# TencentYoutuResearch/ImageMatching-OETR

Hardware: AMD Instinct MI355X
Metric: image-pairs/sec @640x640 (OETR hot path: feature correlation + overlap regression, features resident in HBM) (higher is better)
Workload: dtype f32 (3xf16-split operands, fp32 accumulate); 1 GPU; BASELINE configs[1]: batch=8 pairs/GPU, 640x640 -> 20x20 tokens/image, C=256, 8 enc + 2 dec layers, f32_split_f16; pairs_per_gpu=8, global_pairs=8, streams=3, world_size=1, gpu_max_hw_queues=4, encoder_tile_rows=64, tail_mode=direct form (throughput setting for overlapped streams), parallelism=pairs sharded over 1 rank(s); all-gather of boxes only

## Files before the change

imagematching_oetr_amd/csrc/api.hip:

```cpp
#include <math.h>
#include <stdlib.h>
#include <string.h>

#include <string>
#include <vector>

#include "../../include/oetr_hip.h"
#include "common.h"

using namespace oetr;

constexpr int OETR_PREREDUCE_MIN_TOKENS = 768;
constexpr int OETR_DIRECT_TAIL_MIN_ROWS = 16000;

namespace {

thread_local std::string g_err;

oetr_status fail(oetr_status st, const std::string& msg) {
  g_err = msg;
  return st;
}
oetr_status hip_fail(hipError_t e, const char* what) {
  return fail(OETR_ERR_HIP, std::string(what) + ": " + hipGetErrorString(e));
// ... 91 lines not shown
    "k_decoder", "k_heat_conv", "k_heat_final", "k_size_reg", "k_boxes", "k_decoder_convp",
    "k_heat_combine", "k_neck_proj", "k_neck_conv", "k_neck_out", "k_kv_reduce"};

struct oetr_trace {
  std::vector<hipEvent_t> ev;
  std::vector<int> kid;
  int used = 0;
  int dropped = 0;
};

struct oetr_ctx {
  oetr_trace* trace = nullptr;
  int device = 0;
  int mode = GM_SPLIT;
  int kv_prereduce = -1;
  mutable int dec_fault = 0;
  int dec_split = 0;
  int tail_mode = 0;
  int policy = 0;
  int enc_tile = 0;
  int attn_full = 0;
  int num_cus = 256;
  float* dev = nullptr;
  size_t dev_floats = 0;
  EncLayerDev enc[OETR_N_ENC];
  DecKVDev dkv;
  DecLayerDev dec[OETR_N_DEC];
  const float* qe[2];
  const float *dec_tgt1, *dec_q0, *dec_qkv1;
  HeadsDev heads;
// ... 30 lines not shown

bool make_geom(int n, int hf1, int wf1, int hf2, int wf2, Geom* g) {
  if (n <= 0 || hf1 <= 0 || wf1 <= 0 || hf2 <= 0 || wf2 <= 0) return false;
  const long L1 = (long)hf1 * wf1, L2 = (long)hf2 * wf2;
  if (L1 > OETR_MAX_TOKENS || L2 > OETR_MAX_TOKENS) return false;
  if ((long)n * (L1 + L2) > (1L << 30) / C) return false;
  g->N = n;
  g->L[0] = (int)L1; g->L[1] = (int)L2;
  g->hf[0] = hf1; g->wf[0] = wf1; g->hf[1] = hf2; g->wf[1] = wf2;
  g->nt[0] = (g->L[0] + TM - 1) / TM; g->nt[1] = (g->L[1] + TM - 1) / TM;
  g->row0[0] = 0; g->row0[1] = n * g->L[0];
  g->prow0[0] = 0; g->prow0[1] = g->L[0];
  g->tile0[0] = 0; g->tile0[1] = n * g->nt[0];
  g->ntiles = n * (g->nt[0] + g->nt[1]);
  g->rows = n * (g->L[0] + g->L[1]);
  return true;
}

int encoder_tile_rows(const oetr_ctx* h, const Geom& g) {
  if (!gm_half(h->mode) || h->attn_full) return TM;
  const int want = h->enc_tile;
  if (want == TM || want == 64) return want;
  return g.ntiles > h->num_cus ? 64 : TM;
}
Geom encoder_geom(const Geom& g, int rows) {
  Geom e = g;
  for (int i = 0; i < 2; ++i) e.nt[i] = (g.L[i] + rows - 1) / rows;
  e.tile0[0] = 0; e.tile0[1] = g.N * e.nt[0];
  e.ntiles = g.N * (e.nt[0] + e.nt[1]);
  return e;
}

Workspace carve(const Geom& g, void* base, bool attn_full = false) {
  Workspace w;
  size_t off = 0;
  auto take = [&](size_t floats) {
    float* p = base ? reinterpret_cast<float*>(static_cast<char*>(base) + off) : nullptr;
    off += (floats * sizeof(float) + 255) & ~size_t(255);
    return p;
  };
  const size_t rows = g.rows, nt = g.ntiles;
  w.flags = reinterpret_cast<uint32_t*>(take(OETR_WORKSPACE_STATUS_BYTES / sizeof(float)));
  w.x = take(rows * C);
  w.qp = take((rows + (size_t)2 * g.N * 64) * C);
  w.pos = take((size_t)(g.L[0] + g.L[1]) * C);
// ... 119 lines not shown

oetr_status run_correlation(oetr_ctx* h, const Geom& g, const Workspace& w, const float* feat1,
                            const float* feat2, const float* pos1, const float* pos2,
                            int enc_layers, hipStream_t s, bool with_decoder = true,
                            bool resident = false, const float* mask1 = nullptr,
                            const float* mask2 = nullptr) {
  EncLaunch p;
  memset(&p, 0, sizeof(p));
  if (!resident) {
    p.feat_nchw[0] = feat1; p.feat_nchw[1] = feat2;
    p.pos_nchw[0] = pos1; p.pos_nchw[1] = pos2;
    p.pos_out = w.pos;
  }
  p.tile_rows = encoder_tile_rows(h, g);
  p.g = encoder_geom(g, p.tile_rows);
#ifdef OETR_ABLATE
  { const char* e = getenv("OETR_ABLATE"); p.dbg = e ? atoi(e) : 0; }
#endif
#ifdef OETR_PHASE_TIMING
  {
    static long long* tb = nullptr;
    if (!tb) (void)hipMalloc(&tb, sizeof(long long) * 16 * 65536);
    p.tbuf = tb;
    g_tbuf = tb;
  }
#endif
  p.x = w.x; p.qp = w.qp; p.pos = w.pos;
  p.mask[0] = mask1; p.mask[1] = mask2;
  p.flags = w.flags;
  p.attn_full = h->attn_full;
// ... 1000 lines not shown
    return fail(OETR_ERR_BAD_ARG, "oetr_debug_mfma_rate: NULL output or seconds outside (0, 30]");
  int ndev = 0;
  if (hipGetDeviceCount(&ndev) != hipSuccess || ndev <= 0 || device < 0 || device >= ndev)
    return fail(OETR_ERR_NO_DEVICE, "no HIP device " + std::to_string(device));
  hipDeviceProp_t prop;
  HIP_TRY(hipGetDeviceProperties(&prop, device));
  int prev = 0;
  (void)hipGetDevice(&prev);
  hipError_t e = hipSetDevice(device);
  if (e == hipSuccess) e = measure_mfma_rate(prop.multiProcessorCount, seconds, tflops, static_cast<hipStream_t>(stream));
  (void)hipSetDevice(prev);
  if (e != hipSuccess) return hip_fail(e, "oetr_debug_mfma_rate");
  return OETR_OK;
}

oetr_status oetr_set_state_prereduce(oetr_handle h, int on) {
  if (!h) return fail(OETR_ERR_BAD_ARG, "oetr_set_state_prereduce: NULL handle");
  if (on < -1 || on > 1) return fail(OETR_ERR_BAD_ARG, "oetr_set_state_prereduce: -1 (auto), 0 (off) or 1 (a reduction launch between the encoder launches)");
  h->kv_prereduce = on;
  return OETR_OK;
}

oetr_status oetr_set_attention(oetr_handle h, oetr_attention mode) {
  if (!h) return fail(OETR_ERR_BAD_ARG, "oetr_set_attention: NULL handle");
  if (mode != OETR_ATTENTION_LINEAR && mode != OETR_ATTENTION_FULL)
    return fail(OETR_ERR_BAD_ARG, "oetr_set_attention: unknown mode");
  if (mode == OETR_ATTENTION_FULL && h->policy != 0)
    return fail(OETR_ERR_UNSUPPORTED, "attention 'full' is not built for OETR_DTYPE_F32_SPLIT_QK16");
  if (mode == OETR_ATTENTION_FULL && !gm_f16_range(h->mode) && h->mode != GM_F32)
    return fail(OETR_ERR_UNSUPPORTED, "attention 'full' is built for OETR_DTYPE_F32_SPLIT_F16, OETR_DTYPE_F16 and OETR_DTYPE_F32");
// ... 46 lines not shown
```

imagematching_oetr_amd/csrc/common.h:

```cpp
#pragma once
#include <hip/hip_runtime.h>
#include <stdint.h>

#include <type_traits>

namespace oetr {

constexpr int C = 256;
constexpr int NH = 8;
constexpr int HD = 32;
constexpr int FF = 512;
constexpr int TM = 32;
constexpr int LDA = C + 4;
constexpr int LDH = FF + 4;
constexpr int NTHREADS = 256;
constexpr int KV_FLOATS = NH * HD * HD;
constexpr float LN_EPS = 1e-5f;
constexpr float ATTN_EPS = 1e-6f;
constexpr int MAX_TOKENS = 10000;


#ifdef OETR_ABLATE
#define ABL(flags, bit) (((flags) & (bit)) != 0)
#else
// ... 46 lines not shown
template <> struct SitePolicy<0> {
  static constexpr int Q = SITE_FULL, K = SITE_FULL, V = SITE_FULL, MERGE = SITE_FULL, MLP1 = SITE_FULL,
                       MLP2 = SITE_FULL, DEC_K = SITE_FULL, DEC_V = SITE_FULL;
};
template <> struct SitePolicy<1> {
  static constexpr int Q = SITE_HI, K = SITE_HI, V = SITE_FULL, MERGE = SITE_FULL, MLP1 = SITE_FULL,
                       MLP2 = SITE_FULL, DEC_K = SITE_HI, DEC_V = SITE_FULL;
};
constexpr int N_POLICIES = 2;

constexpr float SPLIT_SCALE = 2048.0f;
constexpr float SPLIT_INV = 1.0f / 2048.0f;
constexpr int LDAH = C + 8;
constexpr int LDHH = FF + 8;

struct Geom {
  int N;
  int L[2];
  int hf[2], wf[2];
  int nt[2];
  int row0[2];
  int prow0[2];
  int tile0[2];
  int ntiles;
  int rows;
};

#if defined(__HIPCC__)

__device__ __forceinline__ float wave_max(float v) {
#pragma unroll
  for (int off = 32; off > 0; off >>= 1) v = fmaxf(v, __shfl_xor(v, off, 64));
  return v;
}

__device__ __forceinline__ int crow(int r, int half) {
  return (r & 3) + 8 * (r >> 2) + 4 * half;
}

__device__ __forceinline__ float exp_neg(float x) {
  const float L2E_HI = 1.4426950216293335f, L2E_LO = 1.9259629911266175e-08f;
// ... 61 lines not shown
  const f32x2 w1 = f32x2{fminf(a1[0], GELU_T), fminf(a1[1], GELU_T)};
  f32x2 q0 = splat2(GELU_Q[GELU_DEG]), q1 = splat2(GELU_Q[GELU_DEG]);
#pragma unroll
  for (int i = GELU_DEG - 1; i >= 0; --i) {
    q0 = __builtin_elementwise_fma(q0, w0, splat2(GELU_Q[i]));
    q1 = __builtin_elementwise_fma(q1, w1, splat2(GELU_Q[i]));
  }
  const f32x2 u0 = __builtin_elementwise_fma(w0, q0, splat2(-1.0f));
  const f32x2 u1 = __builtin_elementwise_fma(w1, q1, splat2(-1.0f));
  f32x4 g;
  g[0] = fmaf(-fabsf(v[0]), __builtin_amdgcn_exp2f(u0[0]), fmaxf(v[0], 0.f));
  g[2] = fmaf(-fabsf(v[2]), __builtin_amdgcn_exp2f(u1[0]), fmaxf(v[2], 0.f));
  g[1] = fmaf(-fabsf(v[1]), __builtin_amdgcn_exp2f(u0[1]), fmaxf(v[1], 0.f));
  g[3] = fmaf(-fabsf(v[3]), __builtin_amdgcn_exp2f(u1[1]), fmaxf(v[3], 0.f));
  return g;
}

__device__ __forceinline__ int xcd_remap(int bid, int nwg) {
  const int q = nwg >> 3, r = nwg & 7, xcd = bid & 7, idx = bid >> 3;
  return (xcd < r ? xcd * (q + 1) : r * (q + 1) + (xcd - r) * q) + idx;
}

template <int NT, int U>
struct GemmRegs {
  f32x4 b[U][NT];
  f32x4 a[U];
};

template <int NT, int U>
__device__ __forceinline__ void gemm_fetch(GemmRegs<NT, U>& r, const float* a_ptr,
                                           const f32x4* const (&w_ptr)[NT], int chunk, unsigned ln) {
#pragma unroll
  for (int u = 0; u < U; ++u)
#pragma unroll
    for (int t = 0; t < NT; ++t) r.b[u][t] = w_ptr[t][(chunk * U + u) * 64 + ln];
// ... 796 lines not shown
```

imagematching_oetr_amd/csrc/encoder.hip:

```cpp
#include <type_traits>

#include "common.h"


#ifndef OETR_SOAK_AMP
#define OETR_SOAK_AMP 0
#endif
#ifndef OETR_SPLIT_STATE
#define OETR_SPLIT_STATE 1
#endif

namespace oetr {

constexpr int S0_OFF = 0;
constexpr int S1_OFF = S0_OFF + TM * LDA;
constexpr int H_OFF = S1_OFF + TILE_FLOATS;
constexpr int KSUM_OFF = H_OFF + HID_FLOATS;
constexpr int Z_OFF = KSUM_OFF + C;
constexpr int LNP_OFF = Z_OFF + TM * NH;
constexpr int SMEM_FLOATS = LNP_OFF + 6 * C;

template <int NW>
struct EncCfg {
  static constexpr int NT = 8 / NW;
// ... 687 lines not shown
          if (lane == 0) p.z0_out[(size_t)slot * NH + h] = z;
        }
      }
    };
    dec_layer(std::integral_constant<int, 0>{});
    dec_layer(std::integral_constant<int, 1>{});
  }
  range_report<MODE>(rg, p.flags);
}

constexpr int LNX_LD = 36;
template <int RTW>
struct E2 {
  static constexpr int RFL = (2 * RTW * LDAH * 2 + 3) / 4;
  static_assert(RFL >= RTW * LDA, "region holds the f32 tile too");
  static constexpr int R1 = 0, R2 = RFL, KSUM = 2 * RFL, LNP = KSUM + C;
  static constexpr int LNX = LNP + 6 * C;
  static constexpr int SMEM = LNX + RTW * LNX_LD;
};

template <int MODE, int NMT = 2, bool MASKED = false>
__device__ __forceinline__ void kv_state_64(const f32x16 (&accK)[NMT], const f32x16 (&accV)[NMT],
                                            int S_len, int nvalid, int half, bool two, f32x16& kv,
                                            float& ksum, Range& rg, const float* msk_s = nullptr) {
  const float inv_len = 1.0f / (float)S_len;
  kv = f32x16{0};
  ksum = 0.f;
  int nv2 = nvalid - 4 * half;
  asm volatile("" : "+v"(nv2));
  if constexpr (MODE == GM_SPLIT && OETR_SPLIT_STATE) {
    f32x16 c1 = {0};
#if OETR_SOAK_AMP & 2
    __builtin_amdgcn_s_setprio(3);
#endif
    auto row_tile = [&](auto MT_) {
      constexpr int mt = decltype(MT_)::value;
#pragma unroll
      for (int st = 0; st < 2; ++st) {
        f32x4 k0, k1, v0, v1;
#pragma unroll
        for (int i = 0; i < 8; ++i) {
          const int r = 8 * st + i;
          float m;
          if constexpr (MASKED) m = msk_s[32 * mt + crow(r, half)];
          else m = 32 * mt + crow(r, 0) < nv2 ? 1.0f : 0.0f;
          const float kk = elu1(accK[mt][r]) * m;
          const float vv = accV[mt][r] * (inv_len * m);
          ksum += kk;
          if (i < 4) { k0[i] = kk; v0[i] = vv; } else { k1[i - 4] = kk; v1[i - 4] = vv; }
        }
        f32x4 ah, al, bh, bl;
        split8(k0, k1, ah, al, rg);
        split8(v0, v1, bh, bl, rg);
        mma16_split3(ah, al, bh, bl, kv, c1);
        __builtin_amdgcn_sched_barrier(0);
      }
    };
    row_tile(std::integral_constant<int, 0>{});
    if constexpr (NMT == 2) {
      if (two) row_tile(std::integral_constant<int, 1>{});
    }
#if OETR_SOAK_AMP & 2
    __builtin_amdgcn_s_setprio(0);
#endif
#pragma unroll
    for (int r = 0; r < 16; ++r) kv[r] = fmaf(c1[r], SPLIT_INV, kv[r]);
  } else {
    auto row_tile = [&](auto MT_) {
      constexpr int mt = decltype(MT_)::value;
      auto operands = [&](int r, float& k, float& v) {
        float m;
        if constexpr (MASKED) m = msk_s[32 * mt + crow(r, half)];
        else m = 32 * mt + crow(r, 0) < nv2 ? 1.0f : 0.0f;
        const float x = accK[mt][r];
        k = (elu1(x)) * m;
        ksum += k;
        v = accV[mt][r] * (inv_len * m);
      };
      float kc, vc;
      operands(0, kc, vc);
#pragma unroll
      for (int r = 0; r < 16; ++r) {
        float kn = 0.f, vn = 0.f;
        if (r + 1 < 16) operands(r + 1, kn, vn);
        kv = __builtin_amdgcn_mfma_f32_32x32x2f32(kc, vc, kv, 0, 0, 0);
        __builtin_amdgcn_sched_barrier(0);
        kc = kn; vc = vn;
// ... 32 lines not shown
  float* lnp_s = smem + L2::LNP;
  float* lnx_s = smem + L2::LNX;
  using WS = WStream2T<MODE, ROWS, NMT>;
  WS ws;
  constexpr int P_MERGE = 0;
  constexpr int P_1A = WS::adv(P_MERGE), P_1B = WS::adv(P_1A), P_2A = WS::adv(P_1B), P_2B = WS::adv(P_2A);
  constexpr int P_T0 = HAS_B ? WS::adv(P_2B) : 0;
  constexpr int P_T1 = WS::adv(P_T0), P_T2 = WS::adv(P_T1), P_T3 = WS::adv(P_T2);

  const Geom& g = p.g;
  const int tid = threadIdx.x, lane = tid & 63, wave = __builtin_amdgcn_readfirstlane(tid >> 6);
  const int half = lane >> 5, col = lane & 31;
  const int wcol = 32 * wave;
  const int lrow = tid / TPR, lpart = tid % TPR;

  const int logical = xcd_remap(blockIdx.x, g.ntiles);
  const int per = g.nt[0] + g.nt[1];
  const int n = logical / per;
  const int rem = logical - n * per;
  const int side = rem >= g.nt[0];
  const int t_idx = side ? rem - g.nt[0] : rem;
  const int L = g.L[side];
  const int l0 = t_idx * RTW;
  const int nvalid = min(RTW, L - l0);
  const size_t row_base = (size_t)g.row0[side] + (size_t)n * L + l0;
  const int slot = g.tile0[side] + n * g.nt[side] + t_idx;
  const size_t qrow_base = (size_t)slot * RTW;
  const bool nchw = !HAS_B && p.feat_nchw[0] != nullptr;
  ws.set_rows(nvalid);
  ws.set_lane(lane);

  stage_ln_params<THREADS, HAS_B, TAIL>(lnp_s, p, tid);
  const f32x4* pos = reinterpret_cast<const f32x4*>(
                         p.pos + (size_t)(g.prow0[side] + l0 + min(lrow, nvalid - 1)) * C) + lpart;

  f32x16 xacc[NMT];
  PHASE_STAMP(p, 0);
  if (!HAS_B) PHASE_STAMP(p, 13);

  if (HAS_B) {
    const int ss = p.b_cross ? 1 - side : side;
    const int S_len = g.L[ss];
    const int nts = p.kv_reduced ? 1 : g.nt[ss];
    const int src_slot0 = p.kv_reduced ? ss * g.N + n : g.tile0[ss] + n * g.nt[ss];

    f32x4 kvB[4];
#pragma unroll
    for (int q = 0; q < 4; ++q) kvB[q] = f32x4{0.f, 0.f, 0.f, 0.f};
    {
      constexpr int KVR = 7;
      const unsigned ln = lane, kl = tid & (C - 1);
      const f32x4* kvp = reinterpret_cast<const f32x4*>(p.kv_in) + ((size_t)src_slot0 * NH + wave) * 256;
      const float* ksp = p.ks_in + (size_t)src_slot0 * C;
      float ks = 0.f;
      if (nts == 1) {
#pragma unroll
        for (int e = 0; e < 4; ++e) kvB[e] = kvp[e * 64 + ln];
        ks = ksp[kl];
      } else
      for (int ti0 = 0; ti0 < nts; ti0 += KVR) {
        f32x4 tmp[KVR][4];
        float kt[KVR];
#pragma unroll
        for (int u = 0; u < KVR; ++u) {
          const int ti = min(ti0 + u, nts - 1);
#pragma unroll
          for (int e = 0; e < 4; ++e) tmp[u][e] = kvp[(size_t)ti * (NH * 256) + e * 64 + ln];
          kt[u] = ksp[(size_t)ti * C + kl];
        }
#pragma unroll
        for (int u = 0; u < KVR; ++u)
          if (ti0 + u < nts) {
#pragma unroll
            for (int e = 0; e < 4; ++e) kvB[e] += tmp[u][e];
            ks += kt[u];
          }
      }
      if (tid < C) ksum_s[tid] = ks;
    }
    ws.template prime<C, P_MERGE, SP::MERGE>(p.b.wmerge, p.b.wmerge_l, wave, 0, lane);
    f32x4 qfrag[NMT][4];
    {
      const f32x4* qf = reinterpret_cast<const f32x4*>(p.qp + qrow_base * C) + (size_t)wave * NMT * 4 * 64;
#pragma unroll
      for (int mt = 0; mt < NMT; ++mt)
#pragma unroll
        for (int u = 0; u < 4; ++u) qfrag[mt][u] = qf[(mt * 4 + u) * 64 + (unsigned)lane];
    }
#pragma unroll
    for (int mt = 0; mt < NMT; ++mt) {
      const float* xr = p.x + (row_base + min(32 * mt + col, nvalid - 1)) * C + wcol + 4 * half;
#pragma unroll
      for (int g4 = 0; g4 < 4; ++g4) {
        const f32x4 v = *reinterpret_cast<const f32x4*>(xr + 8 * g4);
#pragma unroll
        for (int i = 0; i < 4; ++i) xacc[mt][4 * g4 + i] = v[i];
      }
    }
    __syncthreads();
    PHASE_STAMP(p, 1);

    {
      f32x4 kvh[2], kvl[2], ksh[2], ksl[2];
      const float inv_S = 1.0f / (float)S_len;
      (void)inv_S;
      if constexpr (gm_f16_range(MODE)) {
#pragma unroll
        for (int s2 = 0; s2 < 2; ++s2) {
          split8(kvB[2 * s2], kvB[2 * s2 + 1], kvh[s2], kvl[s2], rg);
          const float* kr = ksum_s + wave * HD + 4 * half + 16 * s2;
          split8(*reinterpret_cast<const f32x4*>(kr) * inv_S, *reinterpret_cast<const f32x4*>(kr + 8) * inv_S,
                 ksh[s2], ksl[s2], rg);
        }
      }
#pragma unroll
      for (int mt = 0; mt < NMT; ++mt) {
        if (mt == 1 && !ws.two()) break;
// ... 113 lines not shown
      PHASE_STAMP(p, 7);
      ws.template gemm<FF, P_2B, (TAIL != 2), C, SP::MLP2, SNEXT, XTR>(P1, p.b.w2, p.b.w2_l, wave, 16, lane, xacc,
                                                                       TAIL == 0 ? p.a.wq : p.d.wk[0],
                                                                       TAIL == 0 ? p.a.wq_l : p.d.wk_l[0], wave, 0);
    }
#pragma unroll
    for (int mt = 0; mt < NMT; ++mt)
#pragma unroll
      for (int g4 = 0; g4 < 4; ++g4)
        *reinterpret_cast<f32x4*>(Xf + (32 * mt + col) * LDA + wcol + 8 * g4 + 4 * half) =
            f32x4{xacc[mt][4 * g4], xacc[mt][4 * g4 + 1], xacc[mt][4 * g4 + 2], xacc[mt][4 * g4 + 3]};
    __syncthreads();
#pragma unroll
    for (int i = 0; i < RTW / 8; ++i) {
      const int r = wave + 8 * i;
      if (r < nvalid)
        store16(p.x + (row_base + r) * C, 16u * (unsigned)lane,
                                    *reinterpret_cast<const f32x4*>(Xf + r * LDA + 4 * lane));
    }
    PHASE_STAMP(p, 8);
    if (TAIL == 2) { range_report<MODE>(rg, p.flags); return; }
  } else {
    if (nchw) {
      load_tile_nchw<THREADS, RTW>(R1f, p.feat_nchw[side] + (size_t)n * C * L + l0, L, nvalid, tid);
      load_tile_nchw<THREADS, RTW>(R2f, p.pos_nchw[side] + l0, L, nvalid, tid);
    } else {
#pragma unroll
      for (int i = 0; i < (RTW * C / 4) / THREADS; ++i) {
        const int idx = tid + THREADS * i;
        const int r = idx >> 6, c4 = idx & 63;
        *reinterpret_cast<f32x4*>(R1f + r * LDA + 4 * c4) =
            reinterpret_cast<const f32x4*>(p.x + (row_base + min(r, nvalid - 1)) * C)[c4];
      }
    }
    if (TAIL == 0) ws.template prime<C, P_T0, SP::Q>(p.a.wq, p.a.wq_l, wave, 0, lane);
    if (TAIL == 1) ws.template prime<C, P_T0, SP::DEC_K>(p.d.wk[0], p.d.wk_l[0], wave, 0, lane);
    __syncthreads();
    if (nchw) {
      store_tile_tokens<THREADS, RTW>(p.x + row_base * C, R1f, nvalid, tid);
      if (n == 0) store_tile_tokens<THREADS, RTW>(p.pos_out + (size_t)(g.prow0[side] + l0) * C, R2f, nvalid, tid);
    }
    PHASE_STAMP(p, 14);
  }

  if constexpr (MASKED && TAIL != 2) {
    if (tid < RTW) lnx_s[tid] = tid < nvalid ? p.mask[side][(size_t)n * L + l0 + tid] : 0.f;
  }
  if (TAIL == 0) {
    {
      f32x4 xn[F4], ps[F4];
      if (!HAS_B && nchw) {
        const f32x4* pl = reinterpret_cast<const f32x4*>(R2f + lrow * LDA) + lpart;
#pragma unroll
        for (int i = 0; i < F4; ++i) ps[i] = pl[i * TPR];
      } else {
#pragma unroll
        for (int i = 0; i < F4; ++i) ps[i] = pos[i * TPR];
      }
      ln_rows<TPR, F4>(Xf, tid, xn, 0);
      __syncthreads();
// ... 42 lines not shown
            store16(reinterpret_cast<float*>(qf), ((mt * 4 + 2 * s2) * 64 + (unsigned)lane) * 16u,
                                        __builtin_bit_cast(f32x4, qhi));
            store16(reinterpret_cast<float*>(qf), ((mt * 4 + 2 * s2 + 1) * 64 + (unsigned)lane) * 16u,
                                        __builtin_bit_cast(f32x4, qlo));
          }
        }
      };
      ws.template gemm_epi<C, P_T1, true, C, SP::K, SP::V>(P2, p.a.wk, p.a.wk_l, wave, 0, lane, accK, p.a.wv,
                                                           p.a.wv_l, wave, 0, qepi);
    }
    ws.template gemm<C, P_T2, false, C, SP::V>(P2, p.a.wv, p.a.wv_l, wave, 0, lane, accV, nullptr, nullptr,
                                               0, 0);
    PHASE_STAMP(p, 11);
    f32x16 kv;
    float ksum;
    kv_state_64<MODE, NMT, MASKED>(accK, accV, L, nvalid, half, ws.two(), kv, ksum, rg, lnx_s);
    kv_state_write(kv, ksum, lane, wave, p.kv_out, p.ks_out, slot);
    PHASE_STAMP(p, 12);
  } else if (TAIL == 1) {
    float bias_k[2], bias_v[2];
#pragma unroll
    for (int dl = 0; dl < 2; ++dl) {
      bias_k[dl] = p.d.bk[dl][wcol + col];
      bias_v[dl] = p.d.bv[dl][wcol + col];
    }
    {
      f32x4 xv[F4], ps[F4];
      const f32x4* src = reinterpret_cast<const f32x4*>(Xf + lrow * LDA) + lpart;
#pragma unroll
      for (int i = 0; i < F4; ++i) { xv[i] = src[i * TPR]; ps[i] = pos[i * TPR]; }
      __syncthreads();
#pragma unroll
// ... 3 lines not shown
      }
    }
    __syncthreads();
    auto dec_layer = [&](auto DL) {
      constexpr int dl = decltype(DL)::value;
      constexpr int PK = dl == 0 ? P_T0 : P_T2, PV = dl == 0 ? P_T1 : P_T3;
      f32x16 accK[NMT], accV[NMT];
#pragma unroll
      for (int mt = 0; mt < NMT; ++mt)
#pragma unroll
        for (int r = 0; r < 16; ++r) { accK[mt][r] = bias_k[dl]; accV[mt][r] = bias_v[dl]; }
      ws.template gemm<C, PK, true, C, SP::DEC_K, SP::DEC_V>(P1, p.d.wk[dl], p.d.wk_l[dl], wave, 0, lane, accK,
                                                             p.d.wv[dl], p.d.wv_l[dl], wave, 0);
      ws.template gemm<C, PV, false, C, SP::DEC_V>(P2, p.d.wv[dl], p.d.wv_l[dl], wave, 0, lane, accV, nullptr,
                                                   nullptr, 0, 0);
      f32x16 kv;
      float ksum;
      kv_state_64<MODE, NMT, MASKED>(accK, accV, L, nvalid, half, ws.two(), kv, ksum, rg, lnx_s);
      if constexpr (dl == 1) {
        kv_state_write(kv, ksum, lane, wave, p.dkv1_out, p.dks1_out, slot);
      } else {
        const float* q0 = p.dec_q0 + side * C + wave * HD;
        float a = 0.f;
#pragma unroll
        for (int r = 0; r < 16; ++r) a += q0[crow(r, half)] * kv[r];
        a += __shfl_xor(a, 32, 64);
        float z = q0[col] * ksum;
        z += __shfl_xor(z, 1, 64);
        z += __shfl_xor(z, 2, 64);
        z += __shfl_xor(z, 4, 64);
        z += __shfl_xor(z, 8, 64);
        z += __shfl_xor(z, 16, 64);
        if (half == 0) p.att0_out[(size_t)slot * C + wave * HD + col] = a;
        if (lane == 0) p.z0_out[(size_t)slot * NH + wave] = z;
        ws.template prime<C, P_T2, SP::DEC_K>(p.d.wk[1], p.d.wk_l[1], wave, 0, lane);
      }
    };
    dec_layer(std::integral_constant<int, 0>{});
    dec_layer(std::integral_constant<int, 1>{});
  }
  range_report<MODE>(rg, p.flags);
}

template <bool HAS_B, int TAIL, int MODE, int POL = 0, bool MASKED = false>
__global__ __launch_bounds__(512) void k_encoder64(EncLaunch p) {
  __shared__ __attribute__((aligned(16))) float smem[E2<RT>::SMEM];
  if constexpr (gm_planes(MODE) == 2) {
    const Geom& g = p.g;
    const int logical = xcd_remap(blockIdx.x, g.ntiles);
    const int per = g.nt[0] + g.nt[1];
    const int rem = logical - (logical / per) * per;
    const int side = rem >= g.nt[0];
    const int t_idx = side ? rem - g.nt[0] : rem;
    const int nvalid = min(RT, g.L[side] - t_idx * RT);
    if (__builtin_amdgcn_readfirstlane(nvalid > 32 ? 1 : 0)) encoder64_body<HAS_B, TAIL, MODE, POL, 2, RT, MASKED>(p, smem);
    else encoder64_body<HAS_B, TAIL, MODE, POL, 1, RT, MASKED>(p, smem);
  } else {
    encoder64_body<HAS_B, TAIL, MODE, POL, 0, RT, MASKED>(p, smem);
  }
}

template <bool HAS_B, int TAIL, int MODE, int POL = 0, bool MASKED = false>
__global__ __launch_bounds__(512) void k_encoder32m(EncLaunch p) {
  __shared__ __attribute__((aligned(16))) float smem[E2<TM>::SMEM];
  encoder64_body<HAS_B, TAIL, MODE, POL, 2, TM, MASKED>(p, smem);
}

template <int NOB_TAIL_MAX, class F>
static hipError_t launch_b_tail(bool has_b, int tail, F launch) {
// ... 134 lines not shown
```

imagematching_oetr_amd/hip_engine.py:

```python
import ctypes as C
import os
import time
from pathlib import Path

import torch

_PKG_DIR = Path(__file__).resolve().parent
LIB_PATH = _PKG_DIR / 'csrc' / 'liboetr_hip.so'

N_ENC, N_DEC, D_MODEL, N_HEAD = 8, 2, 256, 8
_f32p = C.POINTER(C.c_float)


class _EncW(C.Structure):
    _fields_ = [(n, _f32p) for n in (
        'q_proj', 'k_proj', 'v_proj', 'merge', 'mlp0', 'mlp2',
        'pre_norm_q_w', 'pre_norm_q_b', 'pre_norm_kv_w', 'pre_norm_kv_b',
        'norm2_w', 'norm2_b')]


class _MhaW(C.Structure):
    _fields_ = [(n, _f32p) for n in (
        'q_proj_w', 'q_proj_b', 'k_proj_w', 'k_proj_b', 'v_proj_w',
        'v_proj_b', 'merge')]
# ... 63 lines not shown
    'oetr_workspace_init', 'oetr_read_flags_async', 'oetr_neck_read_flags_async',
    'oetr_set_state_prereduce', 'oetr_set_tail_mode', 'oetr_set_decoder_split', 'oetr_overlap_frame', 'oetr_read_overlap_image',
    'oetr_forward_masked', 'oetr_feature_correlation_masked', 'oetr_center_estimation_masked',
    'oetr_linear_attention_masked', 'oetr_debug_decoder_fault',
    'oetr_flagslot_device_pointer', 'oetr_forward_flagslot', 'oetr_forward_tokens_flagslot',
    'oetr_neck_forward_tokens_status', 'oetr_debug_mfma_rate')

FLAG_F16_RANGE = 1
FLAG_EXCHANGE = 2
FLAG_INVALID = FLAG_F16_RANGE | FLAG_EXCHANGE
FLAG_PUBLISHED = 0x80000000

BANK_ABI_VERSION = 1
BANK_EXPORTS = ('oetr_bank_abi_version', 'oetr_bank_gather', 'oetr_forward_bank')
FLAG_INDEX = 4

COVIS_ABI_VERSION = 1
COVIS_EXPORTS = ('oetr_covis_abi_version', 'oetr_covis_workspace_bytes', 'oetr_covis_boxes')
COVIS_PARAM_DOUBLES = 40

COVIS_SET_ABI_VERSION = 1
COVIS_SET_EXPORTS = ('oetr_covis_set_abi_version', 'oetr_covis_set_workspace_bytes', 'oetr_covis_boxes_indexed',
                     'oetr_covis_select')
COVIS_MAX_SIDE = 8192

CROP_BATCH_ABI_VERSION = 1
CROP_BATCH_EXPORTS = ('oetr_crop_batch_abi_version', 'oetr_crop_batch_capacity', 'oetr_overlap_crop_batch')


def hot_path_keys():
# ... 94 lines not shown
    lib.oetr_trace_destroy.restype = None
    lib.oetr_trace_destroy.argtypes = [vp]
    lib.oetr_set_trace.restype = i
    lib.oetr_set_trace.argtypes = [vp, vp]
    lib.oetr_trace_summary.restype = i
    lib.oetr_trace_summary.argtypes = [vp, C.POINTER(i), C.POINTER(C.c_char_p),
                                       C.POINTER(i), C.POINTER(C.c_float)]
    lib.oetr_set_encoder_tile.restype = i
    lib.oetr_set_encoder_tile.argtypes = [vp, i]
    lib.oetr_set_attention.restype = i
    lib.oetr_set_attention.argtypes = [vp, i]
    lib.oetr_set_state_prereduce.restype = i
    lib.oetr_set_state_prereduce.argtypes = [vp, i]
    lib.oetr_set_tail_mode.restype = i
    lib.oetr_set_tail_mode.argtypes = [vp, i]
    lib.oetr_set_decoder_split.restype = i
    lib.oetr_set_decoder_split.argtypes = [vp, i]
    lib.oetr_debug_decoder_fault.restype = i
    lib.oetr_debug_decoder_fault.argtypes = [vp, i]
    lib.oetr_neck_create.restype = i
    lib.oetr_neck_create.argtypes = [C.POINTER(_NeckWeights), i, C.POINTER(vp)]
    lib.oetr_neck_destroy.restype = None
    lib.oetr_neck_destroy.argtypes = [vp]
    lib.oetr_neck_workspace_bytes.restype = sz
    lib.oetr_neck_workspace_bytes.argtypes = [vp, i, i, i]
    lib.oetr_neck_forward.restype = i
    lib.oetr_neck_forward.argtypes = [vp, vp, i, i, i, vp, sz, vp, vp]
    lib.oetr_neck_forward_tokens.restype = i
    lib.oetr_neck_forward_tokens.argtypes = [vp, vp, i, i, i, vp, sz, vp, vp]
    lib.oetr_token_buffers.restype = i
# ... 315 lines not shown
        self._ws = {}
        self._flag_reader = _FlagReader()
        self._ws_shape = {}
        self._pos_loaded = {}
        self._enc_tile_set = self._tail_mode_set = self._dec_split_set = 0
        if enc_tile is not None:
            self.set_encoder_tile(enc_tile)
        if attention not in self.ATTENTIONS:
            raise ValueError(f'attention must be one of {sorted(self.ATTENTIONS)}')
        self.attention = attention
        if attention != 'linear':
            _check(self.lib, self.lib.oetr_set_attention(self._h, self.ATTENTIONS[attention]),
                   'oetr_set_attention')
        if os.environ.get('OETR_STATE_PREREDUCE'):
            self.set_state_prereduce(int(os.environ['OETR_STATE_PREREDUCE']))

    __del__ = _destructor('oetr_destroy')

    def set_encoder_tile(self, rows):
        _check(self.lib, self.lib.oetr_set_encoder_tile(self._h, int(rows or 0)),
               'oetr_set_encoder_tile')
        self._enc_tile_set = int(rows or 0)

    def _current_ws(self):
        return self._ws.get(torch.cuda.current_stream(self.device).cuda_stream)

    def set_state_prereduce(self, mode):
        _check(self.lib, self.lib.oetr_set_state_prereduce(self._h, int(mode)), 'oetr_set_state_prereduce')

    def set_tail_mode(self, mode):
        _check(self.lib, self.lib.oetr_set_tail_mode(self._h, int(mode)), 'oetr_set_tail_mode')
        self._tail_mode_set = int(mode)

    def set_decoder_split(self, k):
        _check(self.lib, self.lib.oetr_set_decoder_split(self._h, int(k)), 'oetr_set_decoder_split')
        self._dec_split_set = int(k)

    def debug_decoder_fault(self, on=True):
        _check(self.lib, self.lib.oetr_debug_decoder_fault(self._h, int(bool(on))), 'oetr_debug_decoder_fault')

    def settle_exchange(self):
        ws = self._current_ws()
        if ws is not None:
# ... 594 lines not shown
```

Before: 33870 image-pairs/s.

## Pack both images' ragged encoder tail tiles into one 64-row workgroup

When both images' last 64-row encoder tiles are partly empty and their valid rows fit in half a tile, one workgroup now handles both tails as two row segments. This cuts one workgroup per image pair. It adds segment-aware row indexing and masking in the kv-state reduction, and a second state reduction and attention apply for the B segment. The goal is to stop spending a whole mostly-empty workgroup per tail, at the cost of extra per-tile work and more complex code. It is on by default whenever the shape allows, and a setter API plus an environment variable can force it on or off.

```diff
diff --git a/imagematching_oetr_amd/csrc/api.hip b/imagematching_oetr_amd/csrc/api.hip
--- a/imagematching_oetr_amd/csrc/api.hip
+++ b/imagematching_oetr_amd/csrc/api.hip
@@ -6,6 +6,7 @@
 #include <vector>
 
 #include "../../include/oetr_hip.h"
+#include "../../include/oetr_tail_pairing.h"
 #include "common.h"
 
 using namespace oetr;
@@ -129,6 +130,7 @@
   int device = 0;
   int mode = GM_SPLIT;
   int kv_prereduce = -1;
+  int tail_pairing = -1;
   mutable int dec_fault = 0;
   int dec_split = 0;
   int tail_mode = 0;
@@ -189,6 +191,7 @@
   g->tile0[0] = 0; g->tile0[1] = n * g->nt[0];
   g->ntiles = n * (g->nt[0] + g->nt[1]);
   g->rows = n * (g->L[0] + g->L[1]);
+  g->pair = 0;
   return true;
 }
 
@@ -204,6 +207,11 @@
   e.tile0[0] = 0; e.tile0[1] = g.N * e.nt[0];
   e.ntiles = g.N * (e.nt[0] + e.nt[1]);
   return e;
+}
+bool tails_can_pair(const oetr_ctx* h, const Geom& g, int tile_rows, const float* mask1) {
+  if (tile_rows != RT || h->mode != GM_SPLIT || h->attn_full) return false;
+  if (mask1 && h->policy != 0 && h->policy != 1) return false;
+  return tails_pair(g.L[0], g.L[1], RT);
 }
 
 Workspace carve(const Geom& g, void* base, bool attn_full = false) {
@@ -353,6 +361,13 @@
   }
   p.tile_rows = encoder_tile_rows(h, g);
   p.g = encoder_geom(g, p.tile_rows);
+  {
+    const bool can = tails_can_pair(h, g, p.tile_rows, mask1);
+    if (h->tail_pairing == 1 && !can)
+      return fail(OETR_ERR_BAD_ARG, "oetr_set_tail_pairing(1): this forward cannot pair its tails (64-row tiles, a two-plane "
+                                    "dtype, linear attention, and both images' last tiles ragged with nv1 + nv2 <= 32)");
+    if (h->tail_pairing != 0 && can) set_tail_pairing(p.g, true);
+  }
 #ifdef OETR_ABLATE
   { const char* e = getenv("OETR_ABLATE"); p.dbg = e ? atoi(e) : 0; }
 #endif
@@ -1383,6 +1398,13 @@
   return OETR_OK;
 }
 
+oetr_status oetr_set_tail_pairing(oetr_handle h, int mode) {
+  if (!h) return fail(OETR_ERR_BAD_ARG, "oetr_set_tail_pairing: NULL handle");
+  if (mode < -1 || mode > 1) return fail(OETR_ERR_BAD_ARG, "oetr_set_tail_pairing: -1 (pair when the shape allows), 0 (never) or 1 (required)");
+  h->tail_pairing = mode;
+  return OETR_OK;
+}
+
 oetr_status oetr_set_state_prereduce(oetr_handle h, int on) {
   if (!h) return fail(OETR_ERR_BAD_ARG, "oetr_set_state_prereduce: NULL handle");
   if (on < -1 || on > 1) return fail(OETR_ERR_BAD_ARG, "oetr_set_state_prereduce: -1 (auto), 0 (off) or 1 (a reduction launch between the encoder launches)");
diff --git a/imagematching_oetr_amd/csrc/common.h b/imagematching_oetr_amd/csrc/common.h
--- a/imagematching_oetr_amd/csrc/common.h
+++ b/imagematching_oetr_amd/csrc/common.h
@@ -84,17 +84,9 @@
 constexpr int LDAH = C + 8;
 constexpr int LDHH = FF + 8;
 
-struct Geom {
-  int N;
-  int L[2];
-  int hf[2], wf[2];
-  int nt[2];
-  int row0[2];
-  int prow0[2];
-  int tile0[2];
-  int ntiles;
-  int rows;
-};
+}
+#include "enc_tiles.h"
+namespace oetr {
 
 #if defined(__HIPCC__)
 
@@ -186,11 +178,6 @@
   g[1] = fmaf(-fabsf(v[1]), __builtin_amdgcn_exp2f(u0[1]), fmaxf(v[1], 0.f));
   g[3] = fmaf(-fabsf(v[3]), __builtin_amdgcn_exp2f(u1[1]), fmaxf(v[3], 0.f));
   return g;
-}
-
-__device__ __forceinline__ int xcd_remap(int bid, int nwg) {
-  const int q = nwg >> 3, r = nwg & 7, xcd = bid & 7, idx = bid >> 3;
-  return (xcd < r ? xcd * (q + 1) : r * (q + 1) + (xcd - r) * q) + idx;
 }
 
 template <int NT, int U>
diff --git a/imagematching_oetr_amd/csrc/enc_tiles.h b/imagematching_oetr_amd/csrc/enc_tiles.h
--- /dev/null
+++ b/imagematching_oetr_amd/csrc/enc_tiles.h
@@ -0,0 +1,92 @@
+#pragma once
+
+#if defined(__HIPCC__)
+#define OETR_HD __host__ __device__ __forceinline__
+#else
+#define OETR_HD inline
+#endif
+
+namespace oetr {
+
+struct Geom {
+  int N;
+  int L[2];
+  int hf[2], wf[2];
+  int nt[2];
+  int row0[2];
+  int prow0[2];
+  int tile0[2];
+  int ntiles;
+  int rows;
+  int pair;
+};
+
+OETR_HD int xcd_remap(int bid, int nwg) {
+  const int q = nwg >> 3, r = nwg & 7, xcd = bid & 7, idx = bid >> 3;
+  return (xcd < r ? xcd * (q + 1) : r * (q + 1) + (xcd - r) * q) + idx;
+}
+
+OETR_HD int tail_rows(int L, int rows) { return L - rows * ((L + rows - 1) / rows - 1); }
+OETR_HD bool tails_pair(int L0, int L1, int rows) {
+  const int a = tail_rows(L0, rows), b = tail_rows(L1, rows);
+  return a < rows && b < rows && a + b <= rows / 2;
+}
+OETR_HD int enc_wgs_per_pair(const Geom& g) { return g.nt[0] + g.nt[1] - g.pair; }
+OETR_HD void set_tail_pairing(Geom& g, bool on) {
+  g.pair = on ? 1 : 0;
+  g.ntiles = g.N * enc_wgs_per_pair(g);
+}
+
+struct EncTile {
+  int n, side, t;
+  int nv, nvb, b0;
+};
+OETR_HD EncTile enc_tile(const Geom& g, int logical, int rows) {
+  EncTile e;
+  const int per = enc_wgs_per_pair(g);
+  e.n = logical / per;
+  const int rem = logical - e.n * per;
+  e.nvb = 0;
+  if (g.pair) {
+    const int f0 = g.nt[0] - 1, f1 = g.nt[1] - 1;
+    if (rem < f0) { e.side = 0; e.t = rem; }
+    else if (rem < f0 + f1) { e.side = 1; e.t = rem - f0; }
+    else { e.side = 0; e.t = f0; e.nvb = tail_rows(g.L[1], rows); }
+  } else {
+    e.side = rem >= g.nt[0];
+    e.t = e.side ? rem - g.nt[0] : rem;
+  }
+  const int left = g.L[e.side] - e.t * rows;
+  e.nv = left < rows ? left : rows;
+  e.b0 = (e.nvb > 0 && e.nv <= rows / 4 && e.nvb <= rows / 4) ? rows / 4 : e.nv;
+  return e;
+}
+
+struct EncSegs {
+  int side[2], l0[2], rows[2], slot[2];
+  int b0;
+  int last_b;
+};
+OETR_HD EncSegs enc_segs(const Geom& g, const EncTile& e, int rows) {
+  EncSegs s;
+  s.side[0] = e.side; s.l0[0] = e.t * rows; s.rows[0] = e.nv;
+  s.slot[0] = g.tile0[e.side] + e.n * g.nt[e.side] + e.t;
+  if (e.nvb > 0) {
+    s.side[1] = 1; s.l0[1] = (g.nt[1] - 1) * rows; s.rows[1] = e.nvb;
+    s.slot[1] = g.tile0[1] + e.n * g.nt[1] + g.nt[1] - 1;
+  } else {
+    s.side[1] = e.side; s.l0[1] = s.l0[0] + e.nv - 1; s.rows[1] = 0;
+    s.slot[1] = s.slot[0];
+  }
+  s.b0 = e.b0;
+  s.last_b = s.rows[1] > 0 ? s.rows[1] - 1 : 0;
+  return s;
+}
+OETR_HD int seg_of(const EncSegs& s, int r) { return r >= s.b0; }
+OETR_HD bool seg_row_valid(const EncSegs& s, int r) { return r < s.rows[0] || (r >= s.b0 && r < s.b0 + s.rows[1]); }
+OETR_HD int seg_image_row(const EncSegs& s, int r) {
+  const int d = r - s.b0, a = r < s.rows[0] ? r : s.rows[0] - 1;
+  return r < s.b0 ? s.l0[0] + a : s.l0[1] + (d < s.last_b ? d : s.last_b);
+}
+
+}
diff --git a/imagematching_oetr_amd/csrc/encoder.hip b/imagematching_oetr_amd/csrc/encoder.hip
--- a/imagematching_oetr_amd/csrc/encoder.hip
+++ b/imagematching_oetr_amd/csrc/encoder.hip
@@ -725,20 +725,24 @@
 struct E2 {
   static constexpr int RFL = (2 * RTW * LDAH * 2 + 3) / 4;
   static_assert(RFL >= RTW * LDA, "region holds the f32 tile too");
-  static constexpr int R1 = 0, R2 = RFL, KSUM = 2 * RFL, LNP = KSUM + C;
+  static constexpr int R1 = 0, R2 = RFL, KSUM = 2 * RFL, LNP = KSUM + 2 * C;
   static constexpr int LNX = LNP + 6 * C;
   static constexpr int SMEM = LNX + RTW * LNX_LD;
 };
 
-template <int MODE, int NMT = 2, bool MASKED = false>
+template <int MODE, int NMT = 2, bool MASKED = false, bool SEG = false>
 __device__ __forceinline__ void kv_state_64(const f32x16 (&accK)[NMT], const f32x16 (&accV)[NMT],
                                             int S_len, int nvalid, int half, bool two, f32x16& kv,
-                                            float& ksum, Range& rg, const float* msk_s = nullptr) {
+                                            float& ksum, Range& rg, const float* msk_s = nullptr,
+                                            int row_lo = 0) {
   const float inv_len = 1.0f / (float)S_len;
   kv = f32x16{0};
   ksum = 0.f;
   int nv2 = nvalid - 4 * half;
   asm volatile("" : "+v"(nv2));
+  int lo2 = row_lo - 4 * half;
+  if constexpr (SEG) asm volatile("" : "+v"(lo2));
+  (void)lo2;
   if constexpr (MODE == GM_SPLIT && OETR_SPLIT_STATE) {
     f32x16 c1 = {0};
 #if OETR_SOAK_AMP & 2
@@ -754,6 +758,7 @@
           const int r = 8 * st + i;
           float m;
           if constexpr (MASKED) m = msk_s[32 * mt + crow(r, half)];
+          else if constexpr (SEG) m = (crow(r, 0) < nv2 && crow(r, 0) >= lo2) ? 1.0f : 0.0f;
           else m = 32 * mt + crow(r, 0) < nv2 ? 1.0f : 0.0f;
           const float kk = elu1(accK[mt][r]) * m;
           const float vv = accV[mt][r] * (inv_len * m);
@@ -782,6 +787,7 @@
       auto operands = [&](int r, float& k, float& v) {
         float m;
         if constexpr (MASKED) m = msk_s[32 * mt + crow(r, half)];
+        else if constexpr (SEG) m = (crow(r, 0) < nv2 && crow(r, 0) >= lo2) ? 1.0f : 0.0f;
         else m = 32 * mt + crow(r, 0) < nv2 ? 1.0f : 0.0f;
         const float x = accK[mt][r];
         k = (elu1(x)) * m;
@@ -844,25 +850,38 @@
   const int wcol = 32 * wave;
   const int lrow = tid / TPR, lpart = tid % TPR;
 
+  constexpr bool SEG = ROWS == 1 && RTW == RT;
   const int logical = xcd_remap(blockIdx.x, g.ntiles);
-  const int per = g.nt[0] + g.nt[1];
-  const int n = logical / per;
-  const int rem = logical - n * per;
-  const int side = rem >= g.nt[0];
-  const int t_idx = side ? rem - g.nt[0] : rem;
+  const EncTile et = enc_tile(g, logical, RTW);
+  const int n = et.n, side = et.side, t_idx = et.t;
   const int L = g.L[side];
   const int l0 = t_idx * RTW;
-  const int nvalid = min(RTW, L - l0);
+  const int nvalid = et.nv;
   const size_t row_base = (size_t)g.row0[side] + (size_t)n * L + l0;
   const int slot = g.tile0[side] + n * g.nt[side] + t_idx;
   const size_t qrow_base = (size_t)slot * RTW;
   const bool nchw = !HAS_B && p.feat_nchw[0] != nullptr;
+  const EncSegs sg = enc_segs(g, et, RTW);
+  const bool pairB = SEG && et.nvb > 0;
+  const int sideB = sg.side[1], LB = sideB ? g.L[1] : g.L[0], slotB = sg.slot[1];
+  const int b0 = et.b0;
+  const int nvt = SEG ? b0 + et.nvb : nvalid;
+  auto seg_b = [&](int r) { return SEG && r >= b0; };
+  auto row_valid = [&](int r) { return SEG ? seg_row_valid(sg, r) : r < nvalid; };
+  auto xrow = [&](int r) -> size_t {
+    if constexpr (!SEG) return row_base + min(r, nvalid - 1);
+    else return (seg_b(r) ? (size_t)(sideB ? g.row0[1] : g.row0[0]) + (size_t)n * LB : (size_t)g.row0[side] + (size_t)n * L) +
+                seg_image_row(sg, r);
+  };
+  auto prow = [&](int r) -> int {
+    if constexpr (!SEG) return g.prow0[side] + l0 + min(r, nvalid - 1);
+    else return (seg_b(r) ? (sideB ? g.prow0[1] : g.prow0[0]) : g.prow0[side]) + seg_image_row(sg, r);
+  };
   ws.set_rows(nvalid);
   ws.set_lane(lane);
 
   stage_ln_params<THREADS, HAS_B, TAIL>(lnp_s, p, tid);
-  const f32x4* pos = reinterpret_cast<const f32x4*>(
-                         p.pos + (size_t)(g.prow0[side] + l0 + min(lrow, nvalid - 1)) * C) + lpart;
+  const f32x4* pos = reinterpret_cast<const f32x4*>(p.pos + (size_t)prow(lrow) * C) + lpart;
 
   f32x16 xacc[NMT];
   PHASE_STAMP(p, 0);
@@ -871,13 +890,15 @@
   if (HAS_B) {
     const int ss = p.b_cross ? 1 - side : side;
     const int S_len = g.L[ss];
-    const int nts = p.kv_reduced ? 1 : g.nt[ss];
-    const int src_slot0 = p.kv_reduced ? ss * g.N + n : g.tile0[ss] + n * g.nt[ss];
-
-    f32x4 kvB[4];
-#pragma unroll
-    for (int q = 0; q < 4; ++q) kvB[q] = f32x4{0.f, 0.f, 0.f, 0.f};
-    {
+    const int ssB = p.b_cross ? 1 - sideB : sideB;
+    const int S_lenB = ssB ? g.L[1] : g.L[0];
+
+    auto reduce_state = [&](int src, f32x4 (&kvB)[4], float* ks_dst) {
+      const int nt_src = src ? g.nt[1] : g.nt[0];
+      const int nts = p.kv_reduced ? 1 : nt_src;
+      const int src_slot0 = p.kv_reduced ? src * g.N + n : (src ? g.tile0[1] : g.tile0[0]) + n * nt_src;
+#pragma unroll
+      for (int q = 0; q < 4; ++q) kvB[q] = f32x4{0.f, 0.f, 0.f, 0.f};
       constexpr int KVR = 7;
       const unsigned ln = lane, kl = tid & (C - 1);
       const f32x4* kvp = reinterpret_cast<const f32x4*>(p.kv_in) + ((size_t)src_slot0 * NH + wave) * 256;
@@ -906,8 +927,11 @@
             ks += kt[u];
           }
       }
-      if (tid < C) ksum_s[tid] = ks;
-    }
+      if (tid < C) ks_dst[tid] = ks;
+    };
+    f32x4 kvB[4], kvB2[4];
+    reduce_state(ss, kvB, ksum_s);
+    if constexpr (SEG) reduce_state(ssB, kvB2, ksum_s + C);
     ws.template prime<C, P_MERGE, SP::MERGE>(p.b.wmerge, p.b.wmerge_l, wave, 0, lane);
     f32x4 qfrag[NMT][4];
     {
@@ -919,7 +943,7 @@
     }
 #pragma unroll
     for (int mt = 0; mt < NMT; ++mt) {
-      const float* xr = p.x + (row_base + min(32 * mt + col, nvalid - 1)) * C + wcol + 4 * half;
+      const float* xr = p.x + xrow(32 * mt + col) * C + wcol + 4 * half;
 #pragma unroll
       for (int g4 = 0; g4 < 4; ++g4) {
         const f32x4 v = *reinterpret_cast<const f32x4*>(xr + 8 * g4);
@@ -930,7 +954,45 @@
     __syncthreads();
     PHASE_STAMP(p, 1);
 
-    {
+    if constexpr (SEG) {
+      static_assert(!SEG || gm_f16_range(MODE), "two-segment body: split mode");
+      auto apply = [&](const f32x4 (&kv)[4], const float* ks_row, int s_len, f32x16& macc, float& zs) {
+        f32x4 kvh[2], kvl[2], ksh[2], ksl[2];
+        const float inv_S = 1.0f / (float)s_len;
+#pragma unroll
+        for (int s2 = 0; s2 < 2; ++s2) {
+          split8(kv[2 * s2], kv[2 * s2 + 1], kvh[s2], kvl[s2], rg);
+          const float* kr = ks_row + wave * HD + 4 * half + 16 * s2;
+          split8(*reinterpret_cast<const f32x4*>(kr) * inv_S, *reinterpret_cast<const f32x4*>(kr + 8) * inv_S,
+                 ksh[s2], ksl[s2], rg);
+        }
+        f32x16 zacc = {0}, c1 = {0}, cz = {0};
+        macc = f32x16{0};
+#pragma unroll
+        for (int s2 = 0; s2 < 2; ++s2) {
+          const f32x4 qh = qfrag[0][2 * s2], ql = qfrag[0][2 * s2 + 1];
+          mma16_split3(kvh[s2], kvl[s2], qh, ql, macc, c1);
+          mma16_split3(ksh[s2], ksl[s2], qh, ql, zacc, cz);
+        }
+#pragma unroll
+        for (int r = 0; r < 16; ++r) macc[r] = fmaf(c1[r], SPLIT_INV, macc[r]);
+        zacc[0] = fmaf(cz[0], SPLIT_INV, zacc[0]);
+        const float zdot = zacc[0] * (float)s_len;
+        zs = (float)s_len / (zdot + ATTN_EPS);
+      };
+      f32x16 macc, maccB;
+      float zs, zsB;
+      apply(kvB, ksum_s, S_len, macc, zs);
+      apply(kvB2, ksum_s + C, S_lenB, maccB, zsB);
+      const bool lane_b = col >= b0;
+      zs = lane_b ? zsB : zs;
+#pragma unroll
+      for (int r = 0; r < 16; ++r) macc[r] = lane_b ? maccB[r] : macc[r];
+#pragma unroll
+      for (int g4 = 0; g4 < 4; ++g4)
+        P1.put4(col, wcol + 8 * g4 + 4 * half,
+                f32x4{macc[4 * g4] * zs, macc[4 * g4 + 1] * zs, macc[4 * g4 + 2] * zs, macc[4 * g4 + 3] * zs});
+    } else {
       f32x4 kvh[2], kvl[2], ksh[2], ksl[2];
       const float inv_S = 1.0f / (float)S_len;
       (void)inv_S;
@@ -1074,14 +1136,27 @@
 #pragma unroll
     for (int i = 0; i < RTW / 8; ++i) {
       const int r = wave + 8 * i;
-      if (r < nvalid)
-        store16(p.x + (row_base + r) * C, 16u * (unsigned)lane,
+      if (row_valid(r))
+        store16(p.x + (SEG ? xrow(r) : row_base + r) * C, 16u * (unsigned)lane,
                                     *reinterpret_cast<const f32x4*>(Xf + r * LDA + 4 * lane));
     }
     PHASE_STAMP(p, 8);
     if (TAIL == 2) { range_report<MODE>(rg, p.flags); return; }
   } else {
-    if (nchw) {
+    if (nchw && SEG) {
+      constexpr int CG = THREADS / RTW;
+      const int r = tid % RTW, cg = tid / RTW;
+      const bool sb = seg_b(r);
+      const int li = seg_image_row(sg, r), Ls = sb ? LB : L;
+      const float* fs = (sb ? (sideB ? p.feat_nchw[1] : p.feat_nchw[0]) + (size_t)n * C * LB : p.feat_nchw[side] + (size_t)n * C * L) + li;
+      const float* qs = (sb ? (sideB ? p.pos_nchw[1] : p.pos_nchw[0]) : p.pos_nchw[side]) + li;
+#pragma unroll
+      for (int i = 0; i < C / CG; ++i) {
+        const int c = cg + CG * i;
+        R1f[r * LDA + c] = fs[(size_t)c * Ls];
+        R2f[r * LDA + c] = qs[(size_t)c * Ls];
+      }
+    } else if (nchw) {
       load_tile_nchw<THREADS, RTW>(R1f, p.feat_nchw[side] + (size_t)n * C * L + l0, L, nvalid, tid);
       load_tile_nchw<THREADS, RTW>(R2f, p.pos_nchw[side] + l0, L, nvalid, tid);
     } else {
@@ -1089,21 +1164,40 @@
       for (int i = 0; i < (RTW * C / 4) / THREADS; ++i) {
         const int idx = tid + THREADS * i;
         const int r = idx >> 6, c4 = idx & 63;
-        *reinterpret_cast<f32x4*>(R1f + r * LDA + 4 * c4) =
-            reinterpret_cast<const f32x4*>(p.x + (row_base + min(r, nvalid - 1)) * C)[c4];
+        *reinterpret_cast<f32x4*>(R1f + r * LDA + 4 * c4) = reinterpret_cast<const f32x4*>(p.x + xrow(r) * C)[c4];
       }
     }
     if (TAIL == 0) ws.template prime<C, P_T0, SP::Q>(p.a.wq, p.a.wq_l, wave, 0, lane);
     if (TAIL == 1) ws.template prime<C, P_T0, SP::DEC_K>(p.d.wk[0], p.d.wk_l[0], wave, 0, lane);
     __syncthreads();
-    if (nchw) {
+    if (nchw && SEG) {
+#pragma unroll
+      for (int i = 0; i < (RTW * C / 4) / THREADS; ++i) {
+        const int idx = tid + THREADS * i;
+        const int r = idx >> 6, c4 = idx & 63;
+        if (row_valid(r)) {
+          reinterpret_cast<f32x4*>(p.x + xrow(r) * C)[c4] = *reinterpret_cast<const f32x4*>(R1f + r * LDA + 4 * c4);
+          if (n == 0)
+            reinterpret_cast<f32x4*>(p.pos_out + (size_t)prow(r) * C)[c4] = *reinterpret_cast<const f32x4*>(R2f + r * LDA + 4 * c4);
+        }
+      }
+    } else if (nchw) {
       store_tile_tokens<THREADS, RTW>(p.x + row_base * C, R1f, nvalid, tid);
       if (n == 0) store_tile_tokens<THREADS, RTW>(p.pos_out + (size_t)(g.prow0[side] + l0) * C, R2f, nvalid, tid);
     }
     PHASE_STAMP(p, 14);
   }
 
-  if constexpr (MASKED && TAIL != 2) {
+  if constexpr (MASKED && TAIL != 2 && SEG) {
+    if (tid < RTW) {
+      const bool sb = seg_b(tid);
+      const float* mp = (sb ? (sideB ? p.mask[1] : p.mask[0]) + (size_t)n * LB : p.mask[side] + (size_t)n * L) + seg_image_row(sg, tid);
+      const float m = row_valid(tid) ? *mp : 0.f;
+      lnx_s[tid] = m;
+      lnx_s[RTW + tid] = sb ? 0.f : m;
+      lnx_s[2 * RTW + tid] = sb ? m : 0.f;
+    }
+  } else if constexpr (MASKED && TAIL != 2) {
     if (tid < RTW) lnx_s[tid] = tid < nvalid ? p.mask[side][(size_t)n * L + l0 + tid] : 0.f;
   }
   if (TAIL == 0) {
@@ -1176,8 +1270,15 @@
     PHASE_STAMP(p, 11);
     f32x16 kv;
     float ksum;
+    if constexpr (SEG) {
+      kv_state_64<MODE, NMT, MASKED, true>(accK, accV, L, nvalid, half, false, kv, ksum, rg, lnx_s + RTW, 0);
+      kv_state_write(kv, ksum, lane, wave, p.kv_out, p.ks_out, slot);
+      kv_state_64<MODE, NMT, MASKED, true>(accK, accV, LB, nvt, half, false, kv, ksum, rg, lnx_s + 2 * RTW, b0);
+      if (pairB) kv_state_write(kv, ksum, lane, wave, p.kv_out, p.ks_out, slotB);
+    } else {
     kv_state_64<MODE, NMT, MASKED>(accK, accV, L, nvalid, half, ws.two(), kv, ksum, rg, lnx_s);
     kv_state_write(kv, ksum, lane, wave, p.kv_out, p.ks_out, slot);
+    }
     PHASE_STAMP(p, 12);
   } else if (TAIL == 1) {
     float bias_k[2], bias_v[2];
@@ -1211,25 +1312,38 @@
                                                              p.d.wv[dl], p.d.wv_l[dl], wave, 0);
       ws.template gemm<C, PV, false, C, SP::DEC_V>(P2, p.d.wv[dl], p.d.wv_l[dl], wave, 0, lane, accV, nullptr,
                                                    nullptr, 0, 0);
-      f32x16 kv;
-      float ksum;
-      kv_state_64<MODE, NMT, MASKED>(accK, accV, L, nvalid, half, ws.two(), kv, ksum, rg, lnx_s);
-      if constexpr (dl == 1) {
-        kv_state_write(kv, ksum, lane, wave, p.dkv1_out, p.dks1_out, slot);
-      } else {
-        const float* q0 = p.dec_q0 + side * C + wave * HD;
-        float a = 0.f;
-#pragma unroll
-        for (int r = 0; r < 16; ++r) a += q0[crow(r, half)] * kv[r];
-        a += __shfl_xor(a, 32, 64);
-        float z = q0[col] * ksum;
-        z += __shfl_xor(z, 1, 64);
-        z += __shfl_xor(z, 2, 64);
-        z += __shfl_xor(z, 4, 64);
-        z += __shfl_xor(z, 8, 64);
-        z += __shfl_xor(z, 16, 64);
-        if (half == 0) p.att0_out[(size_t)slot * C + wave * HD + col] = a;
-        if (lane == 0) p.z0_out[(size_t)slot * NH + wave] = z;
+      auto partials = [&](auto SB_) {
+        constexpr bool sb = decltype(SB_)::value;
+        const int sd = sb ? sideB : side, st = sb ? slotB : slot;
+        f32x16 kv;
+        float ksum;
+        if constexpr (SEG)
+          kv_state_64<MODE, NMT, MASKED, true>(accK, accV, sb ? LB : L, sb ? nvt : nvalid, half, false, kv, ksum, rg,
+                                               lnx_s + (sb ? 2 : 1) * RTW, sb ? b0 : 0);
+        else
+          kv_state_64<MODE, NMT, MASKED>(accK, accV, L, nvalid, half, ws.two(), kv, ksum, rg, lnx_s);
+        const bool store = !sb || pairB;
+        if constexpr (dl == 1) {
+          if (store) kv_state_write(kv, ksum, lane, wave, p.dkv1_out, p.dks1_out, st);
+        } else {
+          const float* q0 = p.dec_q0 + sd * C + wave * HD;
+          float a = 0.f;
+#pragma unroll
+          for (int r = 0; r < 16; ++r) a += q0[crow(r, half)] * kv[r];
+          a += __shfl_xor(a, 32, 64);
+          float z = q0[col] * ksum;
+          z += __shfl_xor(z, 1, 64);
+          z += __shfl_xor(z, 2, 64);
+          z += __shfl_xor(z, 4, 64);
+          z += __shfl_xor(z, 8, 64);
+          z += __shfl_xor(z, 16, 64);
+          if (half == 0 && store) p.att0_out[(size_t)st * C + wave * HD + col] = a;
+          if (lane == 0 && store) p.z0_out[(size_t)st * NH + wave] = z;
+        }
+      };
+      partials(std::false_type{});
+      if constexpr (SEG) partials(std::true_type{});
+      if constexpr (dl == 0) {
         ws.template prime<C, P_T2, SP::DEC_K>(p.d.wk[1], p.d.wk_l[1], wave, 0, lane);
       }
     };
@@ -1243,13 +1357,7 @@
 __global__ __launch_bounds__(512) void k_encoder64(EncLaunch p) {
   __shared__ __attribute__((aligned(16))) float smem[E2<RT>::SMEM];
   if constexpr (gm_planes(MODE) == 2) {
-    const Geom& g = p.g;
-    const int logical = xcd_remap(blockIdx.x, g.ntiles);
-    const int per = g.nt[0] + g.nt[1];
-    const int rem = logical - (logical / per) * per;
-    const int side = rem >= g.nt[0];
-    const int t_idx = side ? rem - g.nt[0] : rem;
-    const int nvalid = min(RT, g.L[side] - t_idx * RT);
+    const int nvalid = enc_tile(p.g, xcd_remap(blockIdx.x, p.g.ntiles), RT).nv;
     if (__builtin_amdgcn_readfirstlane(nvalid > 32 ? 1 : 0)) encoder64_body<HAS_B, TAIL, MODE, POL, 2, RT, MASKED>(p, smem);
     else encoder64_body<HAS_B, TAIL, MODE, POL, 1, RT, MASKED>(p, smem);
   } else {
diff --git a/imagematching_oetr_amd/hip_engine.py b/imagematching_oetr_amd/hip_engine.py
--- a/imagematching_oetr_amd/hip_engine.py
+++ b/imagematching_oetr_amd/hip_engine.py
@@ -101,6 +101,8 @@
 BANK_ABI_VERSION = 1
 BANK_EXPORTS = ('oetr_bank_abi_version', 'oetr_bank_gather', 'oetr_forward_bank')
 FLAG_INDEX = 4
+
+TAIL_PAIRING_EXPORTS = ('oetr_set_tail_pairing',)
 
 COVIS_ABI_VERSION = 1
 COVIS_EXPORTS = ('oetr_covis_abi_version', 'oetr_covis_workspace_bytes', 'oetr_covis_boxes')
@@ -225,6 +227,8 @@
     lib.oetr_set_state_prereduce.argtypes = [vp, i]
     lib.oetr_set_tail_mode.restype = i
     lib.oetr_set_tail_mode.argtypes = [vp, i]
+    lib.oetr_set_tail_pairing.restype = i
+    lib.oetr_set_tail_pairing.argtypes = [vp, i]
     lib.oetr_set_decoder_split.restype = i
     lib.oetr_set_decoder_split.argtypes = [vp, i]
     lib.oetr_debug_decoder_fault.restype = i
@@ -570,6 +574,8 @@
                    'oetr_set_attention')
         if os.environ.get('OETR_STATE_PREREDUCE'):
             self.set_state_prereduce(int(os.environ['OETR_STATE_PREREDUCE']))
+        if os.environ.get('OETR_TAIL_PAIRING'):
+            self.set_tail_pairing(int(os.environ['OETR_TAIL_PAIRING']))
 
     __del__ = _destructor('oetr_destroy')
 
@@ -583,6 +589,9 @@
 
     def set_state_prereduce(self, mode):
         _check(self.lib, self.lib.oetr_set_state_prereduce(self._h, int(mode)), 'oetr_set_state_prereduce')
+
+    def set_tail_pairing(self, mode):
+        _check(self.lib, self.lib.oetr_set_tail_pairing(self._h, int(mode)), 'oetr_set_tail_pairing')
 
     def set_tail_mode(self, mode):
         _check(self.lib, self.lib.oetr_set_tail_mode(self._h, int(mode)), 'oetr_set_tail_mode')
diff --git a/include/oetr_tail_pairing.h b/include/oetr_tail_pairing.h
--- /dev/null
+++ b/include/oetr_tail_pairing.h
@@ -0,0 +1,16 @@
+#ifndef OETR_TAIL_PAIRING_H
+#define OETR_TAIL_PAIRING_H
+
+#include "oetr_hip.h"
+
+#ifdef __cplusplus
+extern "C" {
+#endif
+
+oetr_status oetr_set_tail_pairing(oetr_handle h, int mode);
+
+#ifdef __cplusplus
+}
+#endif
+
+#endif
```

Result: faster. 34820 image-pairs/s, median of 4 (+2.8%).
